# Lcrypto/mod-interleaveavx_multithreads-FAID

Measured on AMD Instinct MI355X. Metric: decoded Gb/s @ 10 iters, 50G-PON LDPC; FER match vs AVX512 ref, higher is better.
Workload: dtype i8

## Files before the change

mod-interleaveavx_multithreads-faid_amd/csrc/lnsfaid_swar.h:

```cpp
#ifndef LNSFAID_SWAR_H
#define LNSFAID_SWAR_H

#include <stdint.h>

#if defined(__HIPCC__)
#define SW_DEV 1
#define SW_FN __device__ __forceinline__
#define SW_HD __host__ __device__ __forceinline__
#else
#define SW_DEV 0
#define SW_FN static inline
#define SW_HD static inline
#endif

#define SW_MAX_DEG 24
#ifndef SW_ILP
#define SW_ILP 4
#endif

#if SW_DEV
#define SW_SCHED_FENCE() __builtin_amdgcn_sched_barrier(0)
#else
#define SW_SCHED_FENCE() ((void)0)
#endif

SW_FN uint32_t sw_perm(uint32_t s0, uint32_t s1, uint32_t sel)
{
#if SW_DEV
    return __builtin_amdgcn_perm(s0, s1, sel);
#else
    const uint64_t in = ((uint64_t)s0 << 32) | s1;
    uint32_t r = 0;
    for (int i = 0; i < 4; ++i) {
        const uint32_t s = (sel >> (8 * i)) & 0xffu;
        uint32_t b;
        if (s >= 13) b = 0xff;
        else if (s == 12) b = 0;
        else if (s >= 8) b = ((in >> (8 * (2 * (s - 8) + 1) + 7)) & 1u) ? 0xffu : 0u;
        else b = (uint32_t)(in >> (8 * s)) & 0xffu;
        r |= b << (8 * i);
    }
    return r;
#endif
}
SW_FN uint32_t sw_alignbyte(uint32_t s0, uint32_t s1, uint32_t s2)
{
#if SW_DEV
    return __builtin_amdgcn_alignbyte(s0, s1, s2);
#else
    const uint64_t in = ((uint64_t)s0 << 32) | s1;
    return (uint32_t)(in >> (8 * (s2 & 3u)));
#endif
}
template <int TT>
SW_FN uint32_t sw_bitop3(uint32_t a, uint32_t b, uint32_t c)
{
#if SW_DEV
    return __builtin_amdgcn_bitop3_b32(a, b, c, TT);
#else
    uint32_t r = 0;
    for (int m = 0; m < 8; ++m)
        if ((TT >> m) & 1) r |= ((m & 4) ? a : ~a) & ((m & 2) ? b : ~b) & ((m & 1) ? c : ~c);
    return r;
#endif
}
#define SW_TT_SEL 0xca
#define SW_TT_XOR3 0x96
#define SW_TT_AND3 0x80
#define SW_TT_ANDOR 0xea
#define SW_TT_NANDOR 0xae
#define SW_TT_A_AND_BORC 0xe0
#define SW_TT_XORAND 0x28
#define SW_TT_BFI_C 0xd8
#define SW_TT_ANDNOT_OR 0xf8
#define SW_TT_XNOR_AND 0x82

SW_FN uint32_t sw_vconst(uint32_t k, uint32_t dep = 0u)
{
#if SW_DEV
    uint32_t r;
    asm("v_mov_b32 %0, %1 ; %2" : "=v"(r) : "s"(k), "s"(dep));
    return r;
#else
    (void)dep;
    return k;
#endif
}

#define SW_T2N_LO 0xf900fafbu
#define SW_T2N_HI 0xf8000000u

struct SwK {
    uint32_t c78, c0642, cfc, sel_sign, tt_lo, tt_hi, oh_lo, oh_hi;
    uint32_t cbit[8];
    uint32_t c7f;
    uint32_t c70;
    uint32_t n_lo, n_hi;
    uint32_t c55, c33, c0f;
    uint32_t cm27;
};
SW_FN SwK sw_consts(uint32_t dep = 0u)
{
    SwK k;
    k.c78 = sw_vconst(0x78787878u, dep); k.c0642 = sw_vconst(0x06040200u, dep); k.cfc = sw_vconst(0xfcu, dep);
    k.sel_sign = sw_vconst(0x0b090a08u, dep);
    k.tt_lo = sw_vconst(0x07030100u, dep); k.tt_hi = sw_vconst(0xff3f1f0fu, dep);
    k.oh_lo = sw_vconst(0x08040201u, dep); k.oh_hi = sw_vconst(0x80402010u, dep);
    for (int e = 0; e < 8; ++e) k.cbit[e] = sw_vconst(0x01010101u << e, dep);
    k.c7f = sw_vconst(0x7f7f7f7fu, dep);
    k.c70 = sw_vconst(0x70707070u, dep);
    k.n_lo = sw_vconst(SW_T2N_LO, dep); k.n_hi = sw_vconst(SW_T2N_HI, dep);
    k.c55 = sw_vconst(0x55555555u, dep); k.c33 = sw_vconst(0x33333333u, dep); k.c0f = sw_vconst(0x0f0f0f0fu, dep);
    k.cm27 = sw_vconst(0u - 0x27272727u, dep);
    return k;
}

SW_FN uint32_t sw_mask7(uint32_t x, uint32_t sel_sign) { return sw_perm(x, x << 8, sel_sign); }
#define SW_SEL_SIGN 0x0b090a08u

SW_FN uint32_t sw_popcount7(uint32_t x)
{
    x &= 0x7f7f7f7fu;
    x = x - ((x >> 1) & 0x55555555u);
    x = (x & 0x33333333u) + ((x >> 2) & 0x33333333u);
    return (x + (x >> 4)) & 0x0f0f0f0fu;
}
SW_FN uint32_t sw_therm2num(uint32_t x, uint32_t n_lo, uint32_t n_hi)
{
    const uint32_t a = sw_perm(n_hi, n_lo, x & 0x0f0f0f0fu);
    const uint32_t b = sw_perm(n_hi, n_lo, (x >> 4) & 0x07070707u);
    return a ^ b;
}
SW_FN uint32_t sw_zero_mask(uint32_t x, uint32_t sel_sign) { return ~sw_mask7(x + 0x7f7f7f7fu, sel_sign); }

SW_FN uint32_t sw_gather4(uint32_t g0, uint32_t g1, uint32_t g2, uint32_t g3)
{
    const uint32_t lo = (g1 << 8) | g0, hi = (g3 << 8) | g2;
    return (hi << 16) | lo;
}
SW_FN uint32_t sw_opaque(uint32_t x)
{
#if SW_DEV
    asm("" : "+v"(x));
#endif
    return x;
}
SW_FN uint32_t sw_node_addr(uint32_t x) { return sw_perm(x, x, 0x0c0c0300u) | ((x >> 8) & 3u); }

SW_FN uint32_t sw_table_pick(uint32_t rowmask, uint32_t w_hi, uint32_t w_lo, uint32_t t_hi, uint32_t t_lo, uint32_t m)
{
    return sw_bitop3<SW_TT_SEL>(rowmask, sw_perm(w_hi, w_lo, m), sw_perm(t_hi, t_lo, m));
}
SW_FN uint32_t sw_word_pick(uint32_t nm3, uint32_t nm4, uint32_t x0, uint32_t x1, uint32_t x2)
{
    return sw_bitop3<SW_TT_SEL>(nm4, sw_bitop3<SW_TT_SEL>(nm3, x0, x1), x2);
}
SW_FN void sw_word_deal(uint32_t keep, uint32_t nm3, uint32_t nm4, uint32_t oh[3])
{
    oh[0] = sw_bitop3<SW_TT_AND3>(keep, nm3, nm4);
    oh[1] = sw_bitop3<0x20>(keep, nm3, nm4);
    oh[2] = keep & ~nm4;
}
SW_FN uint32_t sw_argmin_selector(uint32_t w, uint32_t oh8, uint32_t c7f, uint32_t c01, uint32_t c0642)
{
    return sw_bitop3<SW_TT_ANDOR>(((w & oh8) + c7f) >> 7, c01, c0642);
}

struct SwRow {
    uint32_t x[3];
    uint32_t cw;
    uint32_t pa[2];
};

struct SwParams {
    uint32_t lut_lo, lut_hi;
    uint32_t ef_lo, ef_hi;
    int32_t f1, f2;
    int32_t window;
    int32_t ef_tables;
    uint32_t nms_t[4];
    uint32_t oms_lo[2], oms_hi[2];
};

#if SW_DEV
struct SwLds {
    typedef __attribute__((address_space(3))) uint32_t lds_u32;
    typedef __attribute__((address_space(3))) uint8_t lds_u8;
    SW_FN uint32_t rd32(uint32_t a) const { return *(const lds_u32*)(size_t)a; }
    SW_FN void wr32(uint32_t a, uint32_t v) const { *(lds_u32*)(size_t)a = v; }
    SW_FN uint32_t rd8(uint32_t a) const { return *(const lds_u8*)(size_t)a; }
    SW_FN void wr8(uint32_t a, uint32_t v) const { *(lds_u8*)(size_t)a = (uint8_t)v; }
};
#else
struct SwLds {
    uint8_t* base;
    uint32_t rd32(uint32_t a) const { return (uint32_t)base[a] | ((uint32_t)base[a + 1] << 8) | ((uint32_t)base[a + 2] << 16) | ((uint32_t)base[a + 3] << 24); }
    void wr32(uint32_t a, uint32_t v) const { base[a] = (uint8_t)v; base[a + 1] = (uint8_t)(v >> 8); base[a + 2] = (uint8_t)(v >> 16); base[a + 3] = (uint8_t)(v >> 24); }
    uint32_t rd8(uint32_t a) const { return base[a]; }
    void wr8(uint32_t a, uint32_t v) const { base[a] = (uint8_t)v; }
};
#endif

#define SW_BIAS_EN 120

SW_FN uint32_t sw_en_pos(uint32_t v) { return (v & ~255u) | ((v & 63u) << 2) | ((v >> 6) & 3u); }

#define SW_OMS(M) ((M) == 1 || (M) == 3 || (M) == 4)
#define SW_MINSUM(M) ((M) == 0 || SW_OMS(M))

SW_FN int sw_oms_offset(int x, bool window, bool F, int f1, int f2)
{
    if (window && F) {
        if (x < f2) x += 1;
        if (x <= f1) x += 1;
    } else {
        if (x > f1) x -= 1;
        if (x >= f2) x -= 1;
    }
    return x;
}

SW_FN void sw_oms_tables(SwParams& p)
{
    for (int r = 0; r < 2; ++r) {
        uint32_t lo = 0, hi = 0;
        for (int x = 0; x < 8; ++x) {
            const int a = sw_oms_offset(x, r != 0, r != 0, p.f1, p.f2);
            const uint32_t v = (uint32_t)((a > 7 ? 7 : a) & 0xff);
            if (x < 4) lo |= v << (8 * x); else hi |= v << (8 * (x - 4));
        }
        p.oms_lo[r] = lo; p.oms_hi[r] = hi;
    }
}

SW_HD int sw_nms_cste(int m, int factor)
{
    const uint16_t p = (uint16_t)((uint16_t)m * (uint16_t)(int16_t)factor);
    const int16_t q = (int16_t)(p >> 5);
    const int r = q > 127 ? 127 : q;
    return r > 7 ? 7 : r;
}
SW_HD bool sw_nms_fits(int f1, int f2)
{
    if (f1 != f2) return false;
    for (int m = 1; m < 32; ++m)
        if (sw_nms_cste(m, f1) < sw_nms_cste(m - 1, f1)) return false;
    return sw_nms_cste(15, f1) == 7;
}
SW_HD void sw_nms_tables(int factor, uint32_t nms_t[4])
{
    for (int w = 0; w < 4; ++w) nms_t[w] = 0;
    for (int m = 0; m < 16; ++m) {
        const int c = sw_nms_cste(m, factor);
        const uint32_t code = c >= 7 ? 0xffu : ((1u << c) - 1u);
        nms_t[m >> 2] |= code << (8 * (m & 3));
    }
}

struct SwUpd {
    uint32_t za[2], sb[2];
    uint32_t oc[2], hi[2];
};
template <bool MINSUM, bool FLIP = true>
SW_FN SwUpd sw_update_consts(uint32_t c, uint32_t flip, uint32_t bias)
{
    const uint32_t za_p = 0x1f1f1f1fu - bias, za_n = za_p - c;
    const uint32_t sb_p = 0x27272727u - c, sb_n = 0x27272727u;
    const uint32_t oc_p = 0x3f3f3f3fu - c, oc_n = MINSUM ? 0x3f3f3f3fu : oc_p;
    const uint32_t hi_p = 0xbebebebeu - c, hi_n = MINSUM ? 0xbebebebeu : hi_p;
    SwUpd u;
    if (!FLIP) {
        u.za[1] = za_p; u.za[0] = za_n; u.sb[1] = sb_p; u.sb[0] = sb_n; u.oc[1] = oc_p; u.oc[0] = oc_n; u.hi[1] = hi_p; u.hi[0] = hi_n;
        return u;
    }
    u.za[1] = sw_bitop3<SW_TT_SEL>(flip, za_n, za_p); u.za[0] = sw_bitop3<SW_TT_SEL>(flip, za_p, za_n);
    u.sb[1] = sw_bitop3<SW_TT_SEL>(flip, sb_n, sb_p); u.sb[0] = sw_bitop3<SW_TT_SEL>(flip, sb_p, sb_n);
    if (MINSUM) {
        u.oc[1] = sw_bitop3<SW_TT_SEL>(flip, oc_n, oc_p); u.oc[0] = sw_bitop3<SW_TT_SEL>(flip, oc_p, oc_n);
        u.hi[1] = sw_bitop3<SW_TT_SEL>(flip, hi_n, hi_p); u.hi[0] = sw_bitop3<SW_TT_SEL>(flip, hi_p, hi_n);
    } else {
        u.oc[1] = u.oc[0] = oc_p; u.hi[1] = u.hi[0] = hi_p;
    }
    return u;
}
template <bool MINSUM>
SW_FN uint32_t sw_update(uint32_t tb, uint32_t ms, const SwUpd& u, uint32_t sel_sign, uint32_t c80)
{
    const uint32_t za = sw_bitop3<SW_TT_SEL>(ms, u.za[1], u.za[0]);
    const uint32_t sb = sw_bitop3<SW_TT_SEL>(ms, u.sb[1], u.sb[0]);
    const uint32_t oc = MINSUM ? sw_bitop3<SW_TT_SEL>(ms, u.oc[1], u.oc[0]) : u.oc[1];
    const uint32_t hi = MINSUM ? sw_bitop3<SW_TT_SEL>(ms, u.hi[1], u.hi[0]) : u.hi[1];
    const uint32_t zb = tb + za;
    const uint32_t mo = sw_mask7(zb - oc, sel_sign);
    const uint32_t mq = sw_mask7(zb, sel_sign);
    return sw_bitop3<SW_TT_SEL>(mo, hi, sw_bitop3<SW_TT_SEL>(mq, zb, c80)) - sb;
}

struct SwUpd2 {
    uint32_t c, fm, zc, oc, hi;
};
template <bool MINSUM>
SW_FN SwUpd2 sw_update2_consts(uint32_t c, uint32_t fm, uint32_t bias)
{
    SwUpd2 u;
    u.c = c; u.fm = fm;
    u.zc = 0x1f1f1f1fu - bias - c;
    u.oc = MINSUM ? 0u - 0x3f3f3f3fu : 0x3f3f3f3fu - c;
    u.hi = MINSUM ? 0xbebebebeu : 0xbebebebeu - c;
    return u;
}
SW_FN uint32_t sw_upd2_d(uint32_t ms, const SwUpd2& u) { return sw_bitop3<SW_TT_XORAND>(ms, u.fm, u.c); }
SW_FN uint32_t sw_upd2_zb(uint32_t tb, uint32_t d, const SwUpd2& u) { return tb + d + u.zc; }
template <bool MINSUM>
SW_FN uint32_t sw_upd2_out(uint32_t zb, uint32_t d, const SwUpd2& u)
{
    const uint32_t ov = MINSUM ? zb + d + u.oc : zb - u.oc;
    return sw_bitop3<0xcf>(zb, ov, ov);
}
template <bool MINSUM>
SW_FN uint32_t sw_upd2_limit(uint32_t ms, uint32_t d, const SwUpd2& u, uint32_t c80)
{
    return sw_bitop3<SW_TT_ANDOR>(ms, MINSUM ? u.hi - d : u.hi, c80);
}
SW_FN uint32_t sw_upd2_en(uint32_t mout, uint32_t lim, uint32_t zb, uint32_t d, uint32_t cm27) { return sw_bitop3<SW_TT_SEL>(mout, lim, zb) + d + cm27; }
template <bool MINSUM>
SW_FN uint32_t sw_update2(uint32_t tb, uint32_t ms, const SwUpd2& u, uint32_t sel_sign, uint32_t c80, uint32_t cm27)
{
    const uint32_t d = sw_upd2_d(ms, u);
    const uint32_t zb = sw_upd2_zb(tb, d, u);
    const uint32_t mout = sw_mask7(sw_upd2_out<MINSUM>(zb, d, u), sel_sign);
    return sw_upd2_en(mout, sw_upd2_limit<MINSUM>(ms, d, u, c80), zb, d, cm27);
}

SW_FN void sw_min_edge(uint32_t& t1, uint32_t& t2, uint32_t ta[5], uint32_t u, int j)
{
    t2 = sw_bitop3<SW_TT_A_AND_BORC>(t2, t1, u);
    t1 &= u;
#pragma unroll
    for (int b = 0; b < 5; ++b)
        if (((j >> b) & 1) == (b >= 3 ? 1 : 0)) ta[b] &= u;
}
SW_FN void sw_min_quad(uint32_t& t1, uint32_t& t2, uint32_t ta[5], uint32_t v0, uint32_t v1, uint32_t v2, uint32_t v3, int j0)
{
    const uint32_t p0 = v0 & v1, p1 = v2 & v3, q = p0 & p1;
    const uint32_t o0 = v0 | v1, o1 = v2 | v3;
    const uint32_t m2 = sw_bitop3<SW_TT_A_AND_BORC>(o0, p0, p1);
    const uint32_t y = sw_bitop3<SW_TT_A_AND_BORC>(t2, t1, q);
    t2 = sw_bitop3<SW_TT_AND3>(y, m2, o1);
    t1 &= q;
    ta[0] = sw_bitop3<SW_TT_AND3>(ta[0], v0, v2);
    ta[1] &= p0;
    if (((j0 >> 2) & 1) == 0) ta[2] &= q;
    if (((j0 >> 3) & 1) == 1) ta[3] &= q;
    if (((j0 >> 4) & 1) == 1) ta[4] &= q;
}

SW_FN void sw_sign_edge(uint32_t ns[3], uint32_t ms, int j, uint32_t cbit) { ns[j >> 3] = sw_bitop3<SW_TT_ANDNOT_OR>(ns[j >> 3], ms, cbit); }
template <int NJ>
SW_FN void sw_sign_quad(uint32_t ns[3], const uint32_t* ms, int j0, int deg, bool fixed, uint32_t c55, uint32_t c33, uint32_t c0f)
{
    uint32_t m[4];
#pragma unroll
    for (int g = 0; g < 4; ++g) m[g] = (j0 + g < NJ && (fixed || j0 + g < deg)) ? ms[j0 + g < NJ ? j0 + g : 0] : 0u;
    const bool has1 = j0 + 1 < NJ, has2 = j0 + 2 < NJ, has3 = j0 + 3 < NJ;
    const uint32_t a = has1 ? sw_bitop3<SW_TT_SEL>(c55, m[0], m[1]) : m[0];
    const uint32_t b = has3 ? sw_bitop3<SW_TT_SEL>(c55, m[2], m[3]) : m[2];
    const uint32_t q = has2 ? sw_bitop3<SW_TT_SEL>(c33, a, b) : a;
    ns[j0 >> 3] = (j0 & 4) ? sw_bitop3<SW_TT_SEL>(c0f, ns[j0 >> 3], q) : q;
}

SW_FN uint32_t sw_plane_bit(const SwLds& lds, uint32_t era_plane, uint32_t a)
{
    const uint32_t v = (a & ~255u) | ((a >> 2) & 63u) | ((a & 3u) << 6);
    return (lds.rd32(era_plane + ((v >> 5) << 2)) >> (v & 31u)) & 1u;
}

#if SW_DEV
#define SW_MFN __device__ __forceinline__
#else
#define SW_MFN inline
#endif
struct SwNoXch {
    SW_MFN void put(int, uint32_t) const {}
    SW_MFN uint32_t get(int) const { return 0u; }
    SW_MFN void barrier() const {}
};
#define SW_OWN(j) (WAVES == 1 || (((j) & 1) == WAVE))

template <int METHOD, int DEG, bool ERA = false, int WAVES = 1, int WAVE = 0, class Tab, class Xch = SwNoXch>
SW_FN SwRow sw_layer_step(const SwLds& lds, const Tab& tab, const SwParams& p, const SwK& K, uint32_t lane, int deg, SwRow cur, bool fresh,
                          uint32_t rowpar, bool lme, uint32_t era_edges = 0u, uint32_t era_plane = 0u, const Xch& xch = Xch())
{
    static_assert(WAVES == 1 || !ERA, "the erasing variant is built for one wave per codeword only");
    static_assert(!ERA || METHOD == 2, "the erasure exists in Decode_FAID only");
    constexpr int NJ = DEG > 0 ? DEG : SW_MAX_DEG;
    constexpr bool MINSUM = SW_MINSUM(METHOD);
    constexpr bool QUADS = WAVES == 1 && SW_ILP == 4 && DEG > 0;
    constexpr bool NSTREE = WAVES == 1 && SW_ILP == 4;
    const uint32_t c01 = K.cbit[0], c80 = K.cbit[7], c7f = K.c7f, c78 = K.c78, c0642 = K.c0642, cfc = K.cfc, sel_sign = K.sel_sign;
    const uint32_t tid4 = lane << 2;
    uint32_t s4j[NJ], cbj[NJ];
#pragma unroll
    for (int j = 0; j < NJ; ++j) { s4j[j] = (DEG > 0 || j < deg) ? tab.s4(j) : 0u; cbj[j] = (DEG > 0 || j < deg) ? tab.cb256(j) : 0u; }

    const uint32_t c2o = cur.cw & 0x07070707u, c1o = (cur.cw >> 3) & 0x07070707u;
    const uint32_t kp = 0x08080808u - c2o, kn = 0x08080808u + c2o;
    const uint32_t bias = MINSUM ? 0u : 0x06040200u;
    const uint32_t kt_lo = sw_perm(kn, kp, 0x05010400u) + (MINSUM ? 0u : 0x02020000u), kt_hi = sw_perm(kn, kp, 0x07030602u) + (MINSUM ? 0u : 0x06060404u);
    const uint32_t tt_lo = K.tt_lo, tt_hi = K.tt_hi;

    uint32_t padd = 0, psub = 0;
#ifndef SW_EXP_NO_OLDPATCH
    if (!fresh && WAVE == 0) {
        const uint32_t a0 = cur.pa[0] & 0xffffu, a1 = cur.pa[0] >> 16, a2 = cur.pa[1] & 0xffffu, a3 = cur.pa[1] >> 16;
        SW_SCHED_FENCE();
        const uint32_t g0 = lds.rd8(a0), g1 = lds.rd8(a1), g2 = lds.rd8(a2), g3 = lds.rd8(a3);
        const uint32_t mneg = sw_mask7(cur.cw << 1, sel_sign);
        padd = sw_bitop3<SW_TT_SEL>(mneg, c1o, c2o); psub = sw_bitop3<SW_TT_SEL>(mneg, c2o, c1o);
        SW_SCHED_FENCE();
        const uint32_t r = sw_gather4(g0, g1, g2, g3) + padd - psub;
        const uint32_t rh = sw_opaque(r >> 8);
        lds.wr8(a0, r); lds.wr8(a1, rh); lds.wr8(a2, r >> 16); lds.wr8(a3, rh >> 16);
    }
#endif
    if (WAVES == 2) xch.barrier();

    SW_SCHED_FENCE();
    uint32_t tb[NJ], ts[NJ], ms[NJ], ad[NJ], rq[NJ], ld[NJ];
    uint32_t t1 = 0xffffffffu, t2 = 0xffffffffu, ta[5] = { 0xffffffffu, 0xffffffffu, 0xffffffffu, 0xffffffffu, 0xffffffffu };
    uint32_t sx = 0;

#pragma unroll
    for (int j = 0; j < NJ; ++j) {
        if ((DEG > 0 || j < deg) && SW_OWN(j)) {
            const uint32_t x4 = tid4 + s4j[j];
#if SW_DEV
            uint32_t a;
            asm("v_and_or_b32 %0, %1, %2, %3" : "=v"(a) : "v"(x4), "v"(cfc), "s"(cbj[j]));
#else
            const uint32_t a = (x4 & cfc) | cbj[j];
#endif
            ad[j] = a; rq[j] = x4 >> 8;
        }
    }
#pragma unroll
    for (int j = 0; j < NJ; ++j)
        if ((DEG > 0 || j < deg) && SW_OWN(j)) ld[j] = lds.rd32(ad[j]);
    SW_SCHED_FENCE();
#pragma unroll
    for (int j0 = 0; j0 < NJ; j0 += SW_ILP) {
        uint32_t r_[SW_ILP], x_[SW_ILP], s_[SW_ILP], k_[SW_ILP], a_[SW_ILP], i_[SW_ILP], u_[SW_ILP];
#define SW_EDGES(...) _Pragma("unroll") for (int g = 0; g < SW_ILP; ++g) { const int j = j0 + g; if (j < NJ && (DEG > 0 || j < deg) && SW_OWN(j)) { __VA_ARGS__ } }
        _Pragma("unroll") for (int g = SW_ILP - 1; g >= 0; --g) { const int j = j0 + g; if (j < NJ && (DEG > 0 || j < deg) && SW_OWN(j)) r_[g] = sw_alignbyte(ld[j], ld[j], rq[j]); }
        SW_EDGES(x_[g] = (j & 7) ? cur.x[j >> 3] >> (j & 7) : cur.x[j >> 3];)
        SW_EDGES(s_[g] = sw_bitop3<SW_TT_ANDOR>(x_[g], c01, c0642);)
        SW_EDGES(k_[g] = sw_perm(kt_hi, kt_lo, s_[g]);)
        SW_EDGES(tb[j] = r_[g] + k_[g];)
        if (ERA) {
            SW_EDGES(x_[g] &= c01;)
            SW_EDGES(
                if ((era_edges >> j) & 1u) {
                    uint32_t em = 0, match = 0;
                    _Pragma("unroll") for (int k = 0; k < 4; ++k) {
                        const uint32_t a = ad[j] + ((rq[j] + (uint32_t)k) & 3u);
                        em |= sw_plane_bit(lds, era_plane, a) ? (0xffu << (8 * k)) : 0u;
                        const uint32_t pold = (k & 1) ? cur.pa[k >> 1] >> 16 : cur.pa[k >> 1] & 0xffffu;
                        match |= (!fresh && a == pold) ? (0xffu << (8 * k)) : 0u;
                    }
                    const uint32_t en_true = r_[g] - (padd & match) + (psub & match);
                    const uint32_t neg01 = ~((en_true + 0x08080808u) >> 7) & c01;
                    tb[j] = sw_bitop3<SW_TT_SEL>(em, c80 + bias, tb[j]);
                    x_[g] = sw_bitop3<SW_TT_SEL>(em, neg01, x_[g]);
                })
        }
        SW_EDGES(ts[j] = MINSUM ? tb[j] : tb[j] - (ERA ? (x_[g] | c0642) : s_[g]);)
        SW_EDGES(ms[j] = sw_mask7(ts[j], sel_sign);)
        SW_EDGES(a_[g] = sw_bitop3<SW_TT_XOR3>(ts[j], c7f, ms[j]);)
        if (METHOD == 0) {
            uint32_t h_[SW_ILP];
            SW_EDGES(i_[g] = sw_bitop3<SW_TT_NANDOR>(ms[j], c01, K.c70);)
            SW_EDGES(a_[g] = (a_[g] + i_[g]) & 0x8f8f8f8fu;)
            SW_EDGES(h_[g] = sw_mask7(a_[g] << 4, sel_sign);)
            SW_EDGES(a_[g] &= 0x87878787u;)
            SW_EDGES(i_[g] = sw_perm(p.nms_t[3], p.nms_t[2], a_[g]);)
            SW_EDGES(u_[g] = sw_perm(p.nms_t[1], p.nms_t[0], a_[g]);)
            SW_EDGES(u_[g] = sw_bitop3<SW_TT_SEL>(h_[g], i_[g], u_[g]);)
        } else {
            SW_EDGES(i_[g] = MINSUM ? sw_bitop3<SW_TT_NANDOR>(ms[j], c01, c78) : sw_bitop3<SW_TT_XNOR_AND>(x_[g], ms[j], c01);)
            SW_EDGES(a_[g] = (MINSUM ? a_[g] + i_[g] : a_[g] + i_[g] + c78) & 0x87878787u;)
            SW_EDGES(u_[g] = sw_perm(tt_hi, tt_lo, a_[g]);)
        }
        SW_EDGES(
            if (WAVES == 2) sx ^= ts[j];
            else if (j & 1) sx = sw_bitop3<SW_TT_XOR3>(sx, ts[j - 1], ts[j]); else if (j == (DEG > 0 ? DEG : deg) - 1) sx ^= ts[j];)
        if (QUADS) {
            uint32_t v_[4];
            _Pragma("unroll") for (int g = 0; g < 4; ++g) v_[g] = j0 + g < NJ ? u_[g] : 0xffffffffu;
            sw_min_quad(t1, t2, ta, v_[0], v_[1], v_[2], v_[3], j0);
        } else {
            SW_EDGES(sw_min_edge(t1, t2, ta, u_[g], j);)
        }
    }

    if (WAVES == 2) {
        if (WAVE == 1) {
            xch.put(0, t1); xch.put(1, t2); xch.put(2, ta[1]); xch.put(3, ta[2]); xch.put(4, ta[3]); xch.put(5, ta[4]); xch.put(6, sx);
        }
        xch.barrier();
        if (WAVE == 0) {
            const uint32_t o1 = xch.get(0), o2 = xch.get(1);
            ta[0] = t1;
            t2 = sw_bitop3<SW_TT_AND3>(t2, o2, t1 | o1);
            t1 &= o1;
            ta[1] &= xch.get(2); ta[2] &= xch.get(3); ta[3] &= xch.get(4); ta[4] &= xch.get(5);
            sx ^= xch.get(6);
        }
    }
    uint32_t c2n_x = 0, fm_x = 0;
    if (WAVES == 2 && WAVE == 1) {
        xch.barrier();
        c2n_x = xch.get(0); fm_x = xch.get(1);
    }

    const uint32_t n_lo = WAVES == 2 ? SW_T2N_LO : K.n_lo, n_hi = WAVES == 2 ? SW_T2N_HI : K.n_hi;
    const uint32_t min1 = sw_therm2num(t1, n_lo, n_hi), min2 = sw_therm2num(t2, n_lo, n_hi);
    uint32_t c1n, c2n;
    if (METHOD == 0) {
        c2n = min1;
        c1n = min2;
    } else if (SW_OMS(METHOD)) {
        const bool win = p.window && lme;
        const uint32_t w_lo = win ? p.oms_lo[1] : p.oms_lo[0], w_hi = win ? p.oms_hi[1] : p.oms_hi[0];
        c2n = sw_table_pick(rowpar, w_hi, w_lo, p.oms_hi[0], p.oms_lo[0], min1);
        c1n = sw_table_pick(rowpar, w_hi, w_lo, p.oms_hi[0], p.oms_lo[0], min2);
    } else {
        const bool win = (METHOD == 5 || p.ef_tables) && p.window && lme;
        const uint32_t w_lo = win ? p.ef_lo : p.lut_lo, w_hi = win ? p.ef_hi : p.lut_hi;
        c2n = sw_table_pick(rowpar, w_hi, w_lo, p.lut_hi, p.lut_lo, min1);
        c1n = sw_table_pick(rowpar, w_hi, w_lo, p.lut_hi, p.lut_lo, min2);
    }
#if SW_DEV
    asm volatile("" : "+v"(c1n), "+v"(c2n));
#endif
    const uint32_t fm = (WAVES == 2 && WAVE == 1) ? fm_x : sw_mask7(sx, sel_sign);
    if (WAVES == 2 && WAVE == 1) { c2n = c2n_x; c1n = 0u; }

    uint32_t idx = 0, ne7_3 = 0, ne7_4 = 0;
#pragma unroll
    for (int b = 4; b >= 0; --b) {
        const uint32_t dd = sw_bitop3<SW_TT_XORAND>(ta[b], t1, c7f);
        const uint32_t ne7 = dd + c7f;
        const uint32_t ne = ne7 >> (7 - b);
        if (b == 4) ne7_4 = ne7;
        if (b == 3) ne7_3 = ne7;
        if (b == 4) idx = (DEG == 0 && deg <= 16) ? 0u : ~ne & (0x01010101u << 4);
        else if (b == 3) idx = (DEG == 0 && deg <= 8) ? idx : sw_bitop3<0xf2>(idx, ne | (idx >> 1), 0x01010101u << 3);
        else idx = sw_bitop3<SW_TT_ANDNOT_OR>(idx, ne, 0x01010101u << b);
    }

    uint32_t pa[4], sbk[4], gk0 = 0, gk1 = 0, gk2 = 0, gk3 = 0, xb = 0;
    const uint32_t idx4 = idx << 2;
#pragma unroll
#ifdef SW_EXP_NO_ARGMIN
    for (int k = 0; k < 4; ++k) sbk[k] = (cbj[k] << 16) | s4j[k];
#else
    for (int k = 0; k < 4; ++k) sbk[k] = WAVE == 0 ? tab.sb_dyn4((idx4 >> (8 * k)) & 0x7cu) : 0u;
#endif
    SW_SCHED_FENCE();

    const SwUpd2 u2 = sw_update2_consts<MINSUM>(c2n, fm, bias);
    const uint32_t cm27 = WAVES == 2 ? 0u - 0x27272727u : K.cm27;
    uint32_t ns[3] = { 0u, 0u, 0u };
    uint32_t cbit[8];
#pragma unroll
    for (int e = 0; e < 8; ++e) cbit[e] = K.cbit[e];
#define SW_PASS2_ARITH(J0, EN)                                                                                       \
    {                                                                                                                \
        const int j0 = (J0);                                                                                         \
        uint32_t d_[SW_ILP], zb[SW_ILP], mo[SW_ILP], lm[SW_ILP];                                                     \
        SW_EDGES(d_[g] = sw_upd2_d(ms[j], u2);)                                                                      \
        SW_EDGES(zb[g] = sw_upd2_zb(tb[j], d_[g], u2);)                                                              \
        SW_EDGES(mo[g] = sw_upd2_out<MINSUM>(zb[g], d_[g], u2);)                                                     \
        SW_EDGES(mo[g] = sw_mask7(mo[g], sel_sign);)                                              \
        SW_EDGES(lm[g] = sw_upd2_limit<MINSUM>(ms[j], d_[g], u2, c80);)                                              \
        SW_EDGES(EN[g] = sw_upd2_en(mo[g], lm[g], zb[g], d_[g], cm27);)                                              \
        SW_EDGES(EN[g] = sw_alignbyte(EN[g], EN[g], 4u - rq[j]);)                                                    \
        if (NSTREE) sw_sign_quad<NJ>(ns, ms, j0, deg, DEG > 0, K.c55, K.c33, K.c0f);                                 \
        else SW_EDGES(sw_sign_edge(ns, ms[j], j, cbit[j & 7]);)                                                      \
    }
#define SW_PASS2_STORE(J0, EN)                                                                                       \
    {                                                                                                                \
        const int j0 = (J0);                                                                                         \
        SW_EDGES(lds.wr32(ad[j], EN[g]);)                                                                            \
    }
    uint32_t en0[SW_ILP], en1[SW_ILP];
    SW_PASS2_ARITH(0, en0)
    SW_SCHED_FENCE();
#pragma unroll
    for (int k = 0; k < 4; ++k)
        pa[k] = sw_node_addr(tid4 + sbk[k] + ((uint32_t)k << 8));
#ifdef SW_EXP_NO_ARGMIN
    gk0 = ld[0] & 0xffu; gk1 = ld[1] & 0xffu; gk2 = ld[2] & 0xffu; gk3 = ld[3] & 0xffu;
#else
    if (WAVE == 0) { gk0 = lds.rd8(pa[0]); gk1 = lds.rd8(pa[1]); gk2 = lds.rd8(pa[2]); gk3 = lds.rd8(pa[3]); }
#endif
    if (WAVES == 2 && WAVE == 0) {
        xch.put(0, c2n); xch.put(1, fm);
        xch.barrier();
    }
    SW_SCHED_FENCE();
    SW_PASS2_STORE(0, en0)
    if (SW_ILP < NJ) { SW_PASS2_ARITH(SW_ILP, en1) SW_PASS2_STORE(SW_ILP, en1) }
    SW_SCHED_FENCE();
    const uint32_t oh8 = sw_perm(K.oh_hi, K.oh_lo, idx & 0x07070707u);
    const uint32_t nm4 = (DEG == 0 && deg <= 16) ? 0xffffffffu : sw_mask7(ne7_4, sel_sign);
    const uint32_t nm3 = (DEG == 0 && deg <= 8) ? 0xffffffffu : sw_mask7(ne7_3, sel_sign);
    const uint32_t selA = sw_argmin_selector(sw_word_pick(nm3, nm4, cur.x[0], cur.x[1], cur.x[2]), oh8, c7f, c01, c0642);
    if (ERA) xb = selA & c01;
    const uint32_t gb = sw_gather4(gk0, gk1, gk2, gk3);
    uint32_t tbA = gb + sw_perm(kt_hi, kt_lo, selA);
    if (ERA) {
        uint32_t em = 0, match = 0;
#pragma unroll
        for (int k = 0; k < 4; ++k) {
            const uint32_t ik = (idx >> (8 * k)) & 31u;
            if ((era_edges >> ik) & 1u) em |= sw_plane_bit(lds, era_plane, pa[k]) ? (0xffu << (8 * k)) : 0u;
            const uint32_t pold = (k & 1) ? cur.pa[k >> 1] >> 16 : cur.pa[k >> 1] & 0xffffu;
            match |= (!fresh && pa[k] == pold) ? (0xffu << (8 * k)) : 0u;
        }
        const uint32_t en_true = gb - (padd & match) + (psub & match);
        tbA = sw_bitop3<SW_TT_SEL>(em, c80 + bias, tbA);
        xb = sw_bitop3<SW_TT_SEL>(em, ~((en_true + 0x08080808u) >> 7) & c01, xb);
    }
    const uint32_t tsA = MINSUM ? tbA : tbA - (ERA ? (xb | c0642) : selA);
    const uint32_t msA = sw_mask7(tsA, sel_sign);
    const uint32_t negA = ~(msA ^ fm);
    const SwUpd2 u1 = sw_update2_consts<MINSUM>(c1n, fm, bias);
    const uint32_t enA = sw_update2<MINSUM>(tbA, msA, u1, sel_sign, c80, cm27);

#pragma unroll
    for (int jg = 2 * SW_ILP; jg < NJ; jg += SW_ILP) {
        uint32_t en[SW_ILP];
        SW_PASS2_ARITH(jg, en)
        SW_PASS2_STORE(jg, en)
    }
#undef SW_EDGES
#undef SW_PASS2_ARITH
#undef SW_PASS2_STORE
    if (WAVES == 2) {
        if (WAVE == 1) { xch.put(0, ns[0]); xch.put(1, ns[1]); xch.put(2, ns[2]); }
        xch.barrier();
        if (WAVE == 1) { SwRow none = { { 0u, 0u, 0u }, 0u, { 0u, 0u } }; return none; }
        ns[0] |= xch.get(0); ns[1] |= xch.get(1); ns[2] |= xch.get(2);
    }
#ifndef SW_EXP_NO_ARGMIN
    {
        const uint32_t eh = sw_opaque(enA >> 8);
        lds.wr8(pa[0], enA); lds.wr8(pa[1], eh); lds.wr8(pa[2], enA >> 16); lds.wr8(pa[3], eh >> 16);
    }
#endif

    SwRow out;
    const int n = DEG > 0 ? DEG : deg;
#pragma unroll
    for (int g = 0; g < 3; ++g) {
        const int cnt = n - 8 * g < 0 ? 0 : (n - 8 * g > 8 ? 8 : n - 8 * g);
        const uint32_t valid = 0x01010101u * ((1u << cnt) - 1u);
        out.x[g] = ~(ns[g] ^ fm) & valid;
    }
    if (!MINSUM) {
        const uint32_t z2 = sw_zero_mask(c2n, sel_sign), nz1 = ~sw_zero_mask(c1n, sel_sign);
        const uint32_t keep = oh8 & nz1;
        uint32_t oh[3];
        sw_word_deal(keep, nm3, nm4, oh);
#pragma unroll
        for (int g = 0; g < 3; ++g) out.x[g] &= ~z2 | oh[g];
    }
    out.cw = c2n | (c1n << 3) | (negA & 0x40404040u);
    out.pa[0] = pa[0] | (pa[1] << 16);
    out.pa[1] = pa[2] | (pa[3] << 16);
    return out;
}

#endif
```

Baseline: 74.63.

## Compute argmin edge update after stores using exact closed-form for FAID path

For the non-minsum, non-erasure, single-wave path, the argmin-edge gather is moved to after the main pass-2 stores. The edge message is then recomputed with a closed-form saturating update (sw_argmin_exact) from the final sign sums and the c1n-c2n delta. This removes the early LDS read and the selector/table-lookup chain from the critical section. In exchange it reorders LDS reads after the writes and relies on the new formula matching the old update bit for bit.

```diff
diff --git a/mod-interleaveavx_multithreads-faid_amd/csrc/lnsfaid_swar.h b/mod-interleaveavx_multithreads-faid_amd/csrc/lnsfaid_swar.h
--- a/mod-interleaveavx_multithreads-faid_amd/csrc/lnsfaid_swar.h
+++ b/mod-interleaveavx_multithreads-faid_amd/csrc/lnsfaid_swar.h
@@ -166,6 +166,16 @@
     return sw_bitop3<SW_TT_ANDOR>(((w & oh8) + c7f) >> 7, c01, c0642);
 }
 
+SW_FN uint32_t sw_argmin_bit(uint32_t w, uint32_t oh8, uint32_t c7f, uint32_t sel_sign) { return sw_mask7((w & oh8) + c7f, sel_sign); }
+#define SW_ARGMIN_LIMIT 0xa6a6a6a6u
+SW_FN uint32_t sw_argmin_exact(uint32_t a, uint32_t neg, uint32_t delta, uint32_t c0f, uint32_t cm27, uint32_t sel_sign)
+{
+    const uint32_t p15 = sw_bitop3<0x0c>(neg, c0f, c0f);
+    const uint32_t r = (a ^ neg) + delta + p15;
+    const uint32_t over = sw_mask7(r + cm27, sel_sign);
+    return (sw_bitop3<SW_TT_SEL>(over, SW_ARGMIN_LIMIT, r) - p15) ^ neg;
+}
+
 struct SwRow {
     uint32_t x[3];
     uint32_t cw;
@@ -397,6 +407,7 @@
     constexpr bool MINSUM = SW_MINSUM(METHOD);
     constexpr bool QUADS = WAVES == 1 && SW_ILP == 4 && DEG > 0;
     constexpr bool NSTREE = WAVES == 1 && SW_ILP == 4;
+    constexpr bool ASIF = !MINSUM && !ERA && WAVES == 1;
     const uint32_t c01 = K.cbit[0], c80 = K.cbit[7], c7f = K.c7f, c78 = K.c78, c0642 = K.c0642, cfc = K.cfc, sel_sign = K.sel_sign;
     const uint32_t tid4 = lane << 2;
     uint32_t s4j[NJ], cbj[NJ];
@@ -602,7 +613,7 @@
 #ifdef SW_EXP_NO_ARGMIN
     gk0 = ld[0] & 0xffu; gk1 = ld[1] & 0xffu; gk2 = ld[2] & 0xffu; gk3 = ld[3] & 0xffu;
 #else
-    if (WAVE == 0) { gk0 = lds.rd8(pa[0]); gk1 = lds.rd8(pa[1]); gk2 = lds.rd8(pa[2]); gk3 = lds.rd8(pa[3]); }
+    if (WAVE == 0 && !ASIF) { gk0 = lds.rd8(pa[0]); gk1 = lds.rd8(pa[1]); gk2 = lds.rd8(pa[2]); gk3 = lds.rd8(pa[3]); }
 #endif
     if (WAVES == 2 && WAVE == 0) {
         xch.put(0, c2n); xch.put(1, fm);
@@ -615,28 +626,31 @@
     const uint32_t oh8 = sw_perm(K.oh_hi, K.oh_lo, idx & 0x07070707u);
     const uint32_t nm4 = (DEG == 0 && deg <= 16) ? 0xffffffffu : sw_mask7(ne7_4, sel_sign);
     const uint32_t nm3 = (DEG == 0 && deg <= 8) ? 0xffffffffu : sw_mask7(ne7_3, sel_sign);
-    const uint32_t selA = sw_argmin_selector(sw_word_pick(nm3, nm4, cur.x[0], cur.x[1], cur.x[2]), oh8, c7f, c01, c0642);
-    if (ERA) xb = selA & c01;
-    const uint32_t gb = sw_gather4(gk0, gk1, gk2, gk3);
-    uint32_t tbA = gb + sw_perm(kt_hi, kt_lo, selA);
-    if (ERA) {
-        uint32_t em = 0, match = 0;
-#pragma unroll
-        for (int k = 0; k < 4; ++k) {
-            const uint32_t ik = (idx >> (8 * k)) & 31u;
-            if ((era_edges >> ik) & 1u) em |= sw_plane_bit(lds, era_plane, pa[k]) ? (0xffu << (8 * k)) : 0u;
-            const uint32_t pold = (k & 1) ? cur.pa[k >> 1] >> 16 : cur.pa[k >> 1] & 0xffffu;
-            match |= (!fresh && pa[k] == pold) ? (0xffu << (8 * k)) : 0u;
+    uint32_t enA = 0u, negA = 0u;
+    if (!ASIF) {
+        const uint32_t selA = sw_argmin_selector(sw_word_pick(nm3, nm4, cur.x[0], cur.x[1], cur.x[2]), oh8, c7f, c01, c0642);
+        if (ERA) xb = selA & c01;
+        const uint32_t gb = sw_gather4(gk0, gk1, gk2, gk3);
+        uint32_t tbA = gb + sw_perm(kt_hi, kt_lo, selA);
+        if (ERA) {
+            uint32_t em = 0, match = 0;
+#pragma unroll
+            for (int k = 0; k < 4; ++k) {
+                const uint32_t ik = (idx >> (8 * k)) & 31u;
+                if ((era_edges >> ik) & 1u) em |= sw_plane_bit(lds, era_plane, pa[k]) ? (0xffu << (8 * k)) : 0u;
+                const uint32_t pold = (k & 1) ? cur.pa[k >> 1] >> 16 : cur.pa[k >> 1] & 0xffffu;
+                match |= (!fresh && pa[k] == pold) ? (0xffu << (8 * k)) : 0u;
+            }
+            const uint32_t en_true = gb - (padd & match) + (psub & match);
+            tbA = sw_bitop3<SW_TT_SEL>(em, c80 + bias, tbA);
+            xb = sw_bitop3<SW_TT_SEL>(em, ~((en_true + 0x08080808u) >> 7) & c01, xb);
         }
-        const uint32_t en_true = gb - (padd & match) + (psub & match);
-        tbA = sw_bitop3<SW_TT_SEL>(em, c80 + bias, tbA);
-        xb = sw_bitop3<SW_TT_SEL>(em, ~((en_true + 0x08080808u) >> 7) & c01, xb);
-    }
-    const uint32_t tsA = MINSUM ? tbA : tbA - (ERA ? (xb | c0642) : selA);
-    const uint32_t msA = sw_mask7(tsA, sel_sign);
-    const uint32_t negA = ~(msA ^ fm);
-    const SwUpd2 u1 = sw_update2_consts<MINSUM>(c1n, fm, bias);
-    const uint32_t enA = sw_update2<MINSUM>(tbA, msA, u1, sel_sign, c80, cm27);
+        const uint32_t tsA = MINSUM ? tbA : tbA - (ERA ? (xb | c0642) : selA);
+        const uint32_t msA = sw_mask7(tsA, sel_sign);
+        negA = ~(msA ^ fm);
+        const SwUpd2 u1 = sw_update2_consts<MINSUM>(c1n, fm, bias);
+        enA = sw_update2<MINSUM>(tbA, msA, u1, sel_sign, c80, cm27);
+    }
 
 #pragma unroll
     for (int jg = 2 * SW_ILP; jg < NJ; jg += SW_ILP) {
@@ -653,11 +667,19 @@
         if (WAVE == 1) { SwRow none = { { 0u, 0u, 0u }, 0u, { 0u, 0u } }; return none; }
         ns[0] |= xch.get(0); ns[1] |= xch.get(1); ns[2] |= xch.get(2);
     }
+    if (ASIF) {
+        SW_SCHED_FENCE();
+        gk0 = lds.rd8(pa[0]); gk1 = lds.rd8(pa[1]); gk2 = lds.rd8(pa[2]); gk3 = lds.rd8(pa[3]);
+        SW_SCHED_FENCE();
+        negA = ~(sw_argmin_bit(sw_word_pick(nm3, nm4, ns[0], ns[1], ns[2]), oh8, c7f, sel_sign) ^ fm);
+    }
+#define SW_ARGMIN_WRITE()                                                                                            \
+    {                                                                                                                \
+        const uint32_t eh = sw_opaque(enA >> 8);                                \
+        lds.wr8(pa[0], enA); lds.wr8(pa[1], eh); lds.wr8(pa[2], enA >> 16); lds.wr8(pa[3], eh >> 16);                \
+    }
 #ifndef SW_EXP_NO_ARGMIN
-    {
-        const uint32_t eh = sw_opaque(enA >> 8);
-        lds.wr8(pa[0], enA); lds.wr8(pa[1], eh); lds.wr8(pa[2], enA >> 16); lds.wr8(pa[3], eh >> 16);
-    }
+    if (!ASIF) SW_ARGMIN_WRITE()
 #endif
 
     SwRow out;
@@ -679,6 +701,14 @@
     out.cw = c2n | (c1n << 3) | (negA & 0x40404040u);
     out.pa[0] = pa[0] | (pa[1] << 16);
     out.pa[1] = pa[2] | (pa[3] << 16);
+    if (ASIF) {
+        SW_SCHED_FENCE();
+        enA = sw_argmin_exact(sw_gather4(gk0, gk1, gk2, gk3), negA, c1n - c2n, K.c0f, cm27, sel_sign);
+#ifndef SW_EXP_NO_ARGMIN
+        SW_ARGMIN_WRITE()
+#endif
+    }
+#undef SW_ARGMIN_WRITE
     return out;
 }
 
```

Result: no change. 74.81 (median of 6 runs) (+0.2%).
